# albertogp71/qLDPCsim

Hardware: AMD Instinct MI355X
Metric: decoded shots/sec (MS 50-iter, LP118_0) at 1/2/4/8 GPU; achieved HBM GB/s (higher is better)
Workload: dtype f32+f64

## Files before the change

### qldpcsim_amd/csrc/decoder_kernels.hip

```cpp


#include "decode_generic.h"
#include "ms_layered.h"

namespace qldpc {

int ms_flood_max_waves(int kc) { return (kc >= 8 ? 512 : 256) / 64; }

const void* select_ms_layered_kernel(int dc, int g, const char** name) {
#define QLDPC_MSL(D, Gn) if (dc == D && g == Gn) QLDPC_NAMED((&ms_layered_kernel<D, Gn>), "ms_layered_kernel<" #D ", " #Gn ">");
  QLDPC_MSL(7, 0) QLDPC_MSL(8, 0) QLDPC_MSL(7, 1) QLDPC_MSL(8, 1) QLDPC_MSL(7, 2) QLDPC_MSL(8, 2)
  QLDPC_MSL(7, 4) QLDPC_MSL(8, 4) QLDPC_MSL(7, 8) QLDPC_MSL(8, 8)
#undef QLDPC_MSL
  return nullptr;
}

QLDPC_GENERIC_SELECTOR(select_kernel, decode_kernel)

hipError_t launch_decode(const void* kernel, const DecodeArgs& args, int grid, int block,
                         int lds_bytes, hipStream_t stream) {
  void* params[] = {(void*)&args};
  return hipLaunchKernel(kernel, dim3(grid), dim3(block), params, (size_t)lds_bytes, stream);
}

hipError_t configure_kernel(const void* kernel, int lds_bytes) {
  return hipFuncSetAttribute(kernel, hipFuncAttributeMaxDynamicSharedMemorySize, lds_bytes);
}

}
```

### qldpcsim_amd/csrc/ms_flood_qc.h

```cpp

template <typename F, int... I>
__device__ __forceinline__ void static_for_seq(F&& f, std::integer_sequence<int, I...>) {
  (f(std::integral_constant<int, I>{}), ...);
}
template <int N, typename F>
__device__ __forceinline__ void static_for(F&& f) {
  static_for_seq(f, std::make_integer_sequence<int, N>{});
}

template <int N>
__device__ __forceinline__ float row_ror_f32(float x) {
  if constexpr ((N & 15) == 0) {
    return x;
  } else {
    return __builtin_bit_cast(float, __builtin_amdgcn_update_dpp(0, __builtin_bit_cast(int, x), 0x120 + (N & 15),
                                                                 0xf, 0xf, true));
  }
}

template <int N>
__device__ __forceinline__ double row_ror_f64(double x) {
  if constexpr ((N & 15) == 0) {
    return x;
  } else {
    const uint64_t u = __builtin_bit_cast(uint64_t, x);
    const uint32_t lo = (uint32_t)__builtin_amdgcn_update_dpp(0, (int)(uint32_t)u, 0x120 + (N & 15), 0xf, 0xf, true);
    const uint32_t hi =
        (uint32_t)__builtin_amdgcn_update_dpp(0, (int)(uint32_t)(u >> 32), 0x120 + (N & 15), 0xf, 0xf, true);
    return __builtin_bit_cast(double, ((uint64_t)hi << 32) | lo);
  }
}

#ifndef QLDPC_QC_NP
#define QLDPC_QC_NP 34
#endif
template <typename T>
constexpr int qc_np() { return QLDPC_QC_NP < T::NB ? QLDPC_QC_NP : T::NB; }

template <typename T>
constexpr int qc_post64_saving(int c) {
  int zero = 0;
  for (int t = 0; t < T::vdeg[c]; ++t) zero += T::vshift[c][t] == 0;
  return 8 * T::vdeg[c] - 2 * (T::vdeg[c] - zero) - 8;
}
template <typename T>
constexpr bool qc_post64(int c) {
  int rank = 0;
  for (int d = 0; d < T::NB; ++d) {
    const int sd = qc_post64_saving<T>(d), sc = qc_post64_saving<T>(c);
    rank += sd > sc || (sd == sc && d < c);
  }
  return rank < qc_np<T>();
}

template <typename T, int C>
__device__ __forceinline__ double qc_post(double L, const float (&S)[T::NB], const double (&P)[T::NB]) {
  if constexpr (qc_post64<T>(C)) return P[C];
  else return L + (double)S[C];
}

__device__ __forceinline__ uint32_t row_bits(uint64_t b, int rowsh) {
  const uint32_t half = (rowsh & 32) ? (uint32_t)(b >> 32) : (uint32_t)b;
  return (half >> (rowsh & 16)) & 0xffffu;
}

struct RowQueue {
  long long cur, end, rows, batch;
  uint32_t* q;
  uint32_t tk, tlen, seen;
  __device__ __forceinline__ RowQueue(const DecodeArgs& a, long long rows_, int lane)
      : cur(0), end(0), rows(rows_), batch(a.batch), q(a.queue), tk(0), tlen(1), seen(0) {
    if (q) claim(lane);
  }
  __device__ __forceinline__ void claim(int lane) {
    const long long rem = batch - rows - (long long)seen;
    long long len = rem / (4 * rows);
    len = len < 1 ? 1 : (len > 64 ? 64 : len);
    tlen = (uint32_t)len;
    if (lane == 0) tk = atomicAdd(q, tlen);
  }
  __device__ __forceinline__ long long take(int lane) {
    if (cur == end) {
      const uint32_t t = __builtin_amdgcn_readfirstlane(tk);
      seen = t + tlen;
      cur = uniform64(rows + (long long)t);
      end = uniform64(cur + tlen);
    }
    const long long h = cur;
    cur = uniform64(cur + 1);
    if (cur == end) claim(lane);
    return h;
  }
};

template <typename T, int B>
__device__ __forceinline__ uint32_t qc_check(const DecodeArgs& a, double L, float (&S)[T::NB], double (&P)[T::NB],
                                             float (&c2v)[T::MB][T::DC], uint32_t synb, int& fl) {
  constexpr int DC = T::DC;
  static_for<DC>([&](auto E) __attribute__((always_inline)) {
    float& cx = c2v[B][E];
    if constexpr (qc_post64<T>(T::cvar[B][E])) {
      double& px = P[T::cvar[B][E]];
      asm volatile("" : "+v"(px), "+v"(cx));
    } else {
      float& sx = S[T::cvar[B][E]];
      asm volatile("" : "+v"(sx), "+v"(cx));
    }
  });
  double v[DC];
  uint32_t hv[DC], hp[DC];
  static_for<DC>([&](auto E) __attribute__((always_inline)) {
    constexpr int e = E, c = T::cvar[B][e], s = T::cshift[B][e];
    double post;
    if constexpr (qc_post64<T>(c)) post = row_ror_f64<(16 - s) & 15>(P[c]);
    else post = L + (double)row_ror_f32<(16 - s) & 15>(S[c]);
    v[e] = post - (double)c2v[B][e];
    hv[e] = hi_word(v[e]);
    hp[e] = hi_word(post);
  });
  double min1, min2;
  min12_tree<DC>(v, min1, min2);
  const uint32_t ph = xor_tree<DC>(hp);
  const uint32_t sh = xor_tree<DC>(hv);
  double m1 = min1, m2 = min2;
  if (__builtin_expect(ballot((min1 == 0.0) | (min2 == __builtin_inf())) != 0, 0)) {
    m1 = __builtin_isinf(min1) ? 0.0 : min1;
    m2 = __builtin_isinf(min2) ? 0.0 : min2;
    if (m1 == 0.0) fl |= FLAG_MIN_ZERO;
  }
  const uint32_t npm = ((sh >> 31) ^ synb) << 31;
  const uint32_t c1n = opaque_always(__builtin_bit_cast(uint32_t, (float)(a.beta * m1)) ^ npm);
  const uint32_t c2n = opaque_always(__builtin_bit_cast(uint32_t, (float)(a.beta * m2)) ^ npm);
  static_for<DC>([&](auto E) __attribute__((always_inline)) {
    constexpr int e = E;
    const uint32_t c = (__builtin_fabs(v[e]) == min1) ? c2n : c1n;
    c2v[B][e] = __builtin_bit_cast(float, c ^ (hv[e] & 0x80000000u));
  });
  uint32_t unsat = (ph >> 31) ^ synb;
  static_for<DC>([&](auto E) __attribute__((always_inline)) {
    float& cx = c2v[B][E];
    asm volatile("" : "+v"(cx));
  });
  asm volatile("" : "+v"(unsat));
  return unsat;
}

template <int N>
__device__ __forceinline__ uint32_t row_ror_u32(uint32_t x) {
  if constexpr ((N & 15) == 0) {
    return x;
  } else {
    return (uint32_t)__builtin_amdgcn_update_dpp(0, (int)x, 0x120 + (N & 15), 0xf, 0xf, true);
  }
}

template <typename T, int B>
__device__ __forceinline__ uint32_t qc_parity(const uint32_t (&hw)[(T::NB + 31) / 32], uint32_t synb) {
  uint32_t ph = synb;
  static_for<T::DC>([&](auto E) __attribute__((always_inline)) {
    constexpr int e = E, c = T::cvar[B][e], s = T::cshift[B][e];
    ph ^= row_ror_u32<(16 - s) & 15>(hw[c >> 5]) >> (c & 31);
  });
  ph &= 1u;
  asm volatile("" : "+v"(ph));
  return ph;
}

template <typename T, int C>
__device__ __forceinline__ float qc_colsum(const float (&c2v)[T::MB][T::DC]) {
  float s = row_ror_f32<T::vshift[C][0]>(c2v[T::vchk[C][0]][T::vslot[C][0]]);
  static_for<T::vdeg[C] - 1>([&](auto I) __attribute__((always_inline)) {
    constexpr int t = I + 1;
    s = s + row_ror_f32<T::vshift[C][t]>(c2v[T::vchk[C][t]][T::vslot[C][t]]);
  });
  return s;
}

template <typename T>
__device__ __forceinline__ void flood_qc_body(const DecodeArgs& a) {
  constexpr int MB = T::MB, NB = T::NB, DC = T::DC;
  static_assert(qc::kLift == 16, "one DPP row per half-shot");
  const int lane = threadIdx.x & 63;
  const int q = lane >> 4, rowsh = lane & 48;
  const int waves = blockDim.x >> 6;
  const long long rows = 4ll * gridDim.x * waves;
  const long long batch = a.batch;
  constexpr int n = 16 * NB, m = 16 * MB;
  constexpr int wn = (n + 63) / 64;

  float c2v[MB][DC], S[NB];
  double P[NB];
  int it = 0, fl = 0;
  uint32_t synreg = 0;
  long long hs = 4ll * ((long long)blockIdx.x * waves + (threadIdx.x >> 6)) + q;
  RowQueue Q(a, rows, lane);
  bool live = false, fin = true;
  bool conv = false;
  int iters = 0;
  bool started = false;

  for (;;) {
    const uint64_t finb = ballot_b(fin);
    if (finb != 0) {
      if (started) {
        if (fin) {
          const DecodeArgs& f = kargs_fresh();
          int ln = threadIdx.x;
          asm volatile("" : "+v"(ln));
          const int kl = ln & 15, rsh = ln & 48;
          if (f.eh_bits) {
            uint32_t lo = 0, hi = 0;
            static_for<wn>([&](auto W) __attribute__((always_inline)) {
              uint32_t r[4] = {0, 0, 0, 0};
              static_for<4>([&](auto I) __attribute__((always_inline)) {
                constexpr int c = 4 * W + I;
                if constexpr (c < NB) r[I] = row_bits(ballot_b(qc_post<T, c>(a.L, S, P) < 0.0), rsh);
              });
              if (kl == W) lo = r[0] | (r[1] << 16), hi = r[2] | (r[3] << 16);
            });
            if (kl < wn) ((uint64_t*)f.ehat)[hs * wn + kl] = ((uint64_t)hi << 32) | lo;
          } else {
            uint8_t* eo = f.ehat + hs * (long long)n + kl;
            static_for<NB>([&](auto C) __attribute__((always_inline)) {
              eo[16 * C] = (uint8_t)(qc_post<T, C>(a.L, S, P) < 0.0);
            });
          }
          if (f.post) {
            double* po = f.post + hs * (long long)n + kl;
            static_for<NB>([&](auto C) __attribute__((always_inline)) { po[16 * C] = qc_post<T, C>(a.L, S, P); });
          }
          const bool mz = row_bits(ballot_b((fl & FLAG_MIN_ZERO) != 0), rsh) != 0;
          if (kl == 0) {
            f.iters[hs] = iters;
            if (f.flags) f.flags[hs] = (int32_t)((mz ? FLAG_MIN_ZERO : 0) | (conv ? FLAG_CONVERGED : 0));
          }
        }
        if (Q.q) {
#pragma unroll
          for (int r = 0; r < 4; ++r) {
            if ((finb >> (16 * r)) & 1u) {
              const long long h = Q.take(lane);
              if (q == r) hs = h;
            }
          }
        } else if (fin) {
          hs += rows;
        }
      }
      started = true;
      if (fin) {
        live = hs < batch;
        it = 0, synreg = 0;
        if (live) {
          const DecodeArgs& f = kargs_fresh();
          int ln = threadIdx.x;
          asm volatile("" : "+v"(ln));
          const int kl = ln & 15;
          if (f.syn_bits) {
            const uint32_t* row = (const uint32_t*)((const uint64_t*)f.syn + hs * f.wm);
            uint32_t w[(MB + 1) / 2];
#pragma unroll
            for (int i = 0; i < (MB + 1) / 2; ++i) w[i] = row[i];
#pragma unroll
            for (int b = 0; b < MB; ++b) synreg |= ((w[b >> 1] >> (16 * (b & 1) + kl)) & 1u) << b;
          } else {
            const uint8_t* row = f.syn + hs * (long long)m + kl;
            uint32_t w[MB];
#pragma unroll
            for (int b = 0; b < MB; ++b) w[b] = row[16 * b];
#pragma unroll
            for (int b = 0; b < MB; ++b) synreg |= (w[b] & 1u) << b;
          }
        }
        const DecodeArgs& g = kargs_fresh();
        const double vf = (double)g.L32;
        const double av = __builtin_fabs(vf);
        const uint32_t cb = __builtin_bit_cast(uint32_t, (float)(g.beta * av));
        const uint32_t neg = (uint32_t)(vf < 0.0);
        fl = av == 0.0 ? FLAG_MIN_ZERO : 0;
        static_for<MB>([&](auto B) __attribute__((always_inline)) {
          const uint32_t negprod = ((neg * DC) ^ (synreg >> B)) & 1u;
          const float val = __builtin_bit_cast(float, cb | ((neg ^ negprod) << 31));
          static_for<DC>([&](auto E) __attribute__((always_inline)) { c2v[B][E] = val; });
        });
        fin = false;
      }
    }
    if (ballot_b(live) == 0) break;

    if (live) {
      static_for<NB>([&](auto C) __attribute__((always_inline)) {
        if constexpr (qc_post64<T>(C)) {
          double& pc = P[C];
          pc = a.L + (double)qc_colsum<T, C>(c2v);
          asm volatile("" : "+v"(pc));
        } else {
          float& sc = S[C];
          sc = qc_colsum<T, C>(c2v);
          asm volatile("" : "+v"(sc));
        }
      });
      it += 1;
      if (it == a.max_iter) {
        uint32_t hw[(NB + 31) / 32] = {};
        static_for<NB>([&](auto C) __attribute__((always_inline)) {
          hw[C / 32] |= (hi_word(qc_post<T, C>(a.L, S, P)) >> 31) << (C % 32);
        });
        uint32_t un = 0;
        static_for<MB>([&](auto B) __attribute__((always_inline)) {
          un |= qc_parity<T, B>(hw, (synreg >> B) & 1u);
        });
        fin = true, iters = it;
        conv = row_bits(ballot_b(un != 0), rowsh) == 0;
      }
    }
    if (live && !fin) {
      uint32_t unsat = 0;
      static_for<MB>([&](auto B) __attribute__((always_inline)) {
        unsat |= qc_check<T, B>(a, a.L, S, P, c2v, (synreg >> B) & 1u, fl);
      });
      if (row_bits(ballot_b(unsat != 0), rowsh) == 0) fin = true, conv = true, iters = it;
    }
  }
}
```

Baseline: 16.94 million.

## Prefetch next shot's syndrome into LDS and batch work-queue claims

When a half-wave row finishes a shot, the kernel now issues an asynchronous global-to-LDS load of the next shot's bit-packed syndrome and parks the current and next shot indices in a per-wave LDS slot. This hides the syndrome fetch latency behind the current shot's decode. The work queue switches to 32-bit indices with a pending-claim flag, refilling ahead of time with at least 8 entries instead of issuing an atomic exactly when a chunk runs out. Kernel arguments are loaded once into scalar registers per refill, and configure_kernel now subtracts static shared memory from the dynamic LDS request. The cost is extra static LDS, explicit waitcnt barriers, and more complex index bookkeeping.

```diff
diff --git a/qldpcsim_amd/csrc/decoder_kernels.hip b/qldpcsim_amd/csrc/decoder_kernels.hip
--- a/qldpcsim_amd/csrc/decoder_kernels.hip
+++ b/qldpcsim_amd/csrc/decoder_kernels.hip
@@ -24,7 +24,10 @@
 }
 
 hipError_t configure_kernel(const void* kernel, int lds_bytes) {
-  return hipFuncSetAttribute(kernel, hipFuncAttributeMaxDynamicSharedMemorySize, lds_bytes);
+  hipFuncAttributes attr;
+  if (const hipError_t e = hipFuncGetAttributes(&attr, kernel)) return e;
+  const int dyn = lds_bytes - (int)attr.sharedSizeBytes;
+  return hipFuncSetAttribute(kernel, hipFuncAttributeMaxDynamicSharedMemorySize, dyn > 0 ? dyn : 0);
 }
 
 }
diff --git a/qldpcsim_amd/csrc/ms_flood_qc.h b/qldpcsim_amd/csrc/ms_flood_qc.h
--- a/qldpcsim_amd/csrc/ms_flood_qc.h
+++ b/qldpcsim_amd/csrc/ms_flood_qc.h
@@ -65,33 +65,71 @@
 }
 
 struct RowQueue {
-  long long cur, end, rows, batch;
+  long long rows, batch;
   uint32_t* q;
+  uint32_t cur, end;
   uint32_t tk, tlen, seen;
+  bool pend;
   __device__ __forceinline__ RowQueue(const DecodeArgs& a, long long rows_, int lane)
-      : cur(0), end(0), rows(rows_), batch(a.batch), q(a.queue), tk(0), tlen(1), seen(0) {
-    if (q) claim(lane);
-  }
-  __device__ __forceinline__ void claim(int lane) {
+      : rows(rows_), batch(a.batch), q(a.queue), cur(0), end(0), tk(0), tlen(1), seen(0), pend(false) {
+    if (q) refill(lane);
+  }
+  __device__ __forceinline__ void claim(int lane, uint32_t len) {
+    tlen = len;
+    if (lane == 0) tk = atomicAdd(q, tlen);
+    pend = true;
+  }
+  __device__ __forceinline__ uint32_t guided() const {
     const long long rem = batch - rows - (long long)seen;
-    long long len = rem / (4 * rows);
-    len = len < 1 ? 1 : (len > 64 ? 64 : len);
-    tlen = (uint32_t)len;
-    if (lane == 0) tk = atomicAdd(q, tlen);
-  }
-  __device__ __forceinline__ long long take(int lane) {
+    const long long d = 4 * rows;
+    if (rem >= 64 * d) return 64;
+    if (rem >= d && d < (1ll << 26)) return (uint32_t)rem / (uint32_t)d;
+    return 1;
+  }
+  __device__ __forceinline__ void refill(int lane) {
+    const uint32_t left = end - cur;
+    if (!pend && left < 4) {
+      const uint32_t g = guided();
+      claim(lane, g > 8 - left ? g : 8 - left);
+    }
+  }
+  __device__ __forceinline__ uint32_t take() {
     if (cur == end) {
       const uint32_t t = __builtin_amdgcn_readfirstlane(tk);
+      pend = false;
       seen = t + tlen;
-      cur = uniform64(rows + (long long)t);
-      end = uniform64(cur + tlen);
-    }
-    const long long h = cur;
-    cur = uniform64(cur + 1);
-    if (cur == end) claim(lane);
-    return h;
+      cur = t;
+      end = t + tlen;
+    }
+    return cur++;
   }
 };
+
+struct HandArgs {
+  const uint8_t* syn;
+  uint8_t* ehat;
+  int32_t* iters;
+  double* post;
+  int32_t* flags;
+  double beta;
+  float L32;
+  int syn_bits, eh_bits, wm;
+};
+__device__ __forceinline__ HandArgs hand_args() {
+  const DecodeArgs& k = kargs_fresh();
+  HandArgs f = {k.syn, k.ehat, k.iters, k.post, k.flags, k.beta, k.L32, k.syn_bits, k.eh_bits, k.wm};
+  asm volatile(""
+               : "+s"(f.syn), "+s"(f.ehat), "+s"(f.iters), "+s"(f.post), "+s"(f.flags), "+s"(f.beta), "+s"(f.L32),
+                 "+s"(f.syn_bits), "+s"(f.eh_bits), "+s"(f.wm));
+  return f;
+}
+
+typedef uint32_t u32x4 __attribute__((ext_vector_type(4)));
+template <int WAVES>
+__device__ __forceinline__ uint32_t syn_park() {
+  __shared__ __attribute__((aligned(16))) uint32_t park[WAVES][64];
+  return lds_addr(&park[0][0]);
+}
 
 template <typename T, int B>
 __device__ __forceinline__ uint32_t qc_check(const DecodeArgs& a, double L, float (&S)[T::NB], double (&P)[T::NB],
@@ -181,18 +219,19 @@
   constexpr int MB = T::MB, NB = T::NB, DC = T::DC;
   static_assert(qc::kLift == 16, "one DPP row per half-shot");
   const int lane = threadIdx.x & 63;
-  const int q = lane >> 4, rowsh = lane & 48;
+  const int rowsh = lane & 48;
   const int waves = blockDim.x >> 6;
   const long long rows = 4ll * gridDim.x * waves;
   const long long batch = a.batch;
   constexpr int n = 16 * NB, m = 16 * MB;
   constexpr int wn = (n + 63) / 64;
+  constexpr int NW = (MB + 1) / 2, NQ = (NW + 3) / 4;
+  static_assert(NW <= 8, "a syndrome row fits the first half of its 64-byte slot (dwords 8 .. 11: the indices)");
 
   float c2v[MB][DC], S[NB];
   double P[NB];
   int it = 0, fl = 0;
   uint32_t synreg = 0;
-  long long hs = 4ll * ((long long)blockIdx.x * waves + (threadIdx.x >> 6)) + q;
   RowQueue Q(a, rows, lane);
   bool live = false, fin = true;
   bool conv = false;
@@ -202,12 +241,72 @@
   for (;;) {
     const uint64_t finb = ballot_b(fin);
     if (finb != 0) {
+      const HandArgs f = hand_args();
+      int ln = threadIdx.x;
+      asm volatile("" : "+v"(ln));
+      const int kl = ln & 15, rsh = ln & 48;
+      const uint32_t wslot = syn_park<ms_flood_max_threads<(16 * MB + 63) / 64>() / 64>() + 256 * (ln >> 6);
+      const uint32_t slot = wslot + 4 * rsh;
+      long long hs = 0, hnew = 4ll * ((long long)blockIdx.x * waves + (ln >> 6)) + (rsh >> 4);
+      if (started && fin) {
+        const u32x4 x = *QLDPC_LDS(const u32x4, slot + 32);
+        hs = (long long)(((uint64_t)x.y << 32) | x.x);
+        hnew = (long long)(((uint64_t)x.w << 32) | x.z);
+      }
+      const bool parked = started && f.syn_bits != 0;
+      if (fin) {
+        live = hnew < batch;
+        it = 0, synreg = 0;
+        if (live) {
+          if (parked) {
+            asm volatile("s_waitcnt vmcnt(0)" ::: "memory");
+            uint32_t w[4 * NQ];
+#pragma unroll
+            for (int i = 0; i < NQ; ++i) {
+              const u32x4 x = *QLDPC_LDS(const u32x4, slot + 16 * i);
+              w[4 * i] = x.x, w[4 * i + 1] = x.y, w[4 * i + 2] = x.z, w[4 * i + 3] = x.w;
+            }
+            asm volatile("s_waitcnt lgkmcnt(0)" : "+v"(w[0]) : : "memory");
+#pragma unroll
+            for (int b = 0; b < MB; ++b) synreg |= ((w[b >> 1] >> (16 * (b & 1) + kl)) & 1u) << b;
+          } else if (f.syn_bits) {
+            const uint32_t* row = (const uint32_t*)((const uint64_t*)f.syn + hnew * f.wm);
+            uint32_t w[NW];
+#pragma unroll
+            for (int i = 0; i < NW; ++i) w[i] = row[i];
+#pragma unroll
+            for (int b = 0; b < MB; ++b) synreg |= ((w[b >> 1] >> (16 * (b & 1) + kl)) & 1u) << b;
+          } else {
+            const uint8_t* row = f.syn + hnew * (long long)m + kl;
+            uint32_t w[MB];
+#pragma unroll
+            for (int b = 0; b < MB; ++b) w[b] = row[16 * b];
+#pragma unroll
+            for (int b = 0; b < MB; ++b) synreg |= (w[b] & 1u) << b;
+          }
+        }
+      }
+      long long hnext = hnew + rows;
+      if (Q.q) {
+#pragma unroll
+        for (int r = 0; r < 4; ++r) {
+          if ((finb >> (16 * r)) & 1u) {
+            const uint32_t t = Q.take();
+            if (rsh == 16 * r) hnext = rows + (long long)t;
+          }
+        }
+      }
+      if (fin) {
+        *QLDPC_LDS(u32x4, slot + 32) = u32x4{(uint32_t)(uint64_t)hnew, (uint32_t)((uint64_t)hnew >> 32),
+                                             (uint32_t)(uint64_t)hnext, (uint32_t)((uint64_t)hnext >> 32)};
+        if (f.syn_bits && hnext < batch && kl < NW) {
+          const uint32_t* src = (const uint32_t*)((const uint64_t*)f.syn + hnext * f.wm) + kl;
+          __builtin_amdgcn_global_load_lds((const __attribute__((address_space(1))) uint32_t*)(uintptr_t)src,
+                                           QLDPC_LDS(uint32_t, wslot), 4, 0, 0);
+        }
+      }
       if (started) {
         if (fin) {
-          const DecodeArgs& f = kargs_fresh();
-          int ln = threadIdx.x;
-          asm volatile("" : "+v"(ln));
-          const int kl = ln & 15, rsh = ln & 48;
           if (f.eh_bits) {
             uint32_t lo = 0, hi = 0;
             static_for<wn>([&](auto W) __attribute__((always_inline)) {
@@ -235,47 +334,13 @@
             if (f.flags) f.flags[hs] = (int32_t)((mz ? FLAG_MIN_ZERO : 0) | (conv ? FLAG_CONVERGED : 0));
           }
         }
-        if (Q.q) {
-#pragma unroll
-          for (int r = 0; r < 4; ++r) {
-            if ((finb >> (16 * r)) & 1u) {
-              const long long h = Q.take(lane);
-              if (q == r) hs = h;
-            }
-          }
-        } else if (fin) {
-          hs += rows;
-        }
-      }
+      }
+      if (Q.q) Q.refill(lane);
       started = true;
       if (fin) {
-        live = hs < batch;
-        it = 0, synreg = 0;
-        if (live) {
-          const DecodeArgs& f = kargs_fresh();
-          int ln = threadIdx.x;
-          asm volatile("" : "+v"(ln));
-          const int kl = ln & 15;
-          if (f.syn_bits) {
-            const uint32_t* row = (const uint32_t*)((const uint64_t*)f.syn + hs * f.wm);
-            uint32_t w[(MB + 1) / 2];
-#pragma unroll
-            for (int i = 0; i < (MB + 1) / 2; ++i) w[i] = row[i];
-#pragma unroll
-            for (int b = 0; b < MB; ++b) synreg |= ((w[b >> 1] >> (16 * (b & 1) + kl)) & 1u) << b;
-          } else {
-            const uint8_t* row = f.syn + hs * (long long)m + kl;
-            uint32_t w[MB];
-#pragma unroll
-            for (int b = 0; b < MB; ++b) w[b] = row[16 * b];
-#pragma unroll
-            for (int b = 0; b < MB; ++b) synreg |= (w[b] & 1u) << b;
-          }
-        }
-        const DecodeArgs& g = kargs_fresh();
-        const double vf = (double)g.L32;
+        const double vf = (double)f.L32;
         const double av = __builtin_fabs(vf);
-        const uint32_t cb = __builtin_bit_cast(uint32_t, (float)(g.beta * av));
+        const uint32_t cb = __builtin_bit_cast(uint32_t, (float)(f.beta * av));
         const uint32_t neg = (uint32_t)(vf < 0.0);
         fl = av == 0.0 ? FLAG_MIN_ZERO : 0;
         static_for<MB>([&](auto B) __attribute__((always_inline)) {
```

Measured after the change: 16.95 million, median of 6. No clear change (+0.1%).
